# erlgo/openair4G

Hardware: AMD Instinct MI355X
Metric: DL subframes/sec (20 MHz, 2x2, 64-QAM) (higher is better)
Workload: dtype int16; 1 GPU; dlsim 20 MHz 2x2 TM3 (LARGE_CDD) 64-QAM MCS19x2CW, 2x14 IDFT-2048; config_id=C3, global_batch=8192, subframe_index=7, full_grid=False, parallelism=subframe-sharded x1

## Files before the change

include/oai4g.h:

```cpp
#ifndef OAI4G_H
#define OAI4G_H

#include <stddef.h>
#include <stdint.h>

#ifdef __cplusplus
extern "C" {
#endif

#define OAI4G_LTE_NULL 2
#define OAI4G_NSOFT 1827072
#define OAI4G_MAX_SEGMENTS 16
#define OAI4G_MAX_CHANNEL_BITS (14 * 1200 * 6)
#define OAI4G_D_BYTES (96 + 12 + 3 + 3 * 6144)
#define OAI4G_W_BYTES (3 * 6144 + 96)

enum {
  OAI4G_SISO = 0,
  OAI4G_ALAMOUTI = 1,
  OAI4G_LARGE_CDD = 2,
  OAI4G_UNIFORM_PRECODING11 = 3,
  OAI4G_UNIFORM_PRECODING1m1 = 4,
  OAI4G_UNIFORM_PRECODING1j = 5,
  OAI4G_UNIFORM_PRECODING1mj = 6,
// ... 58 lines not shown

typedef struct {
  uint16_t rnti;
  uint8_t current_harq_pid;
  uint8_t Mdlharq;
  uint8_t Kmimo;
  int16_t sqrt_rho_a;
  int16_t sqrt_rho_b;
  oai4g_dl_harq_t *harq_processes[8];
} oai4g_dlsch_t;

int oai4g_init(void);
const char *oai4g_last_error(void);
int oai4g_device_name(char *buf, int len);

int oai4g_init_frame_parms(oai4g_frame_parms_t *fp, uint16_t N_RB_DL, uint16_t Nid_cell, uint8_t Ncp,
                           uint8_t nb_antennas_tx, uint8_t mode1_flag, uint8_t frame_type);
uint8_t oai4g_get_Qm(uint8_t mcs);
int oai4g_get_G(const oai4g_frame_parms_t *fp, uint16_t nb_rb, const uint32_t *rb_alloc, uint8_t mod_order,
                uint8_t Nl, uint8_t num_pdcch_symbols, int frame, uint8_t subframe);
uint8_t oai4g_get_Qm_ul(uint8_t mcs);
uint8_t oai4g_get_I_TBS(uint8_t mcs);
uint8_t oai4g_get_I_TBS_UL(uint8_t mcs);
uint32_t oai4g_tbs_bits(uint8_t I_TBS, uint16_t nb_rb);
uint32_t oai4g_get_TBS_DL(uint8_t mcs, uint16_t nb_rb);
uint32_t oai4g_get_TBS_UL(uint8_t mcs, uint16_t nb_rb);
oai4g_dlsch_t *oai4g_new_dlsch(uint8_t Kmimo, uint8_t Mdlharq, uint8_t N_RB_DL);
void oai4g_free_dlsch(oai4g_dlsch_t *dlsch);
uint32_t oai4g_lte_gold_generic(uint32_t *x1, uint32_t *x2, uint8_t reset);
int oai4g_qpp_fold32(uint32_t K, uint32_t *s, uint16_t *tab);
int oai4g_rsc_scan_rows(uint32_t q, uint32_t rows[6]);
int oai4g_rm_pair_schedule(uint32_t C, uint32_t n0, const uint32_t nt[2], const uint32_t wrapt[2],
                           uint32_t *pairs, uint32_t *pair0);
int oai4g_mod_item_map(uint32_t item, uint32_t ips, uint32_t lz, uint32_t per, uint32_t *sf, uint32_t *l,
                       uint32_t *pair);
uint8_t oai4g_get_pmi(uint8_t N_RB_DL, uint8_t mimo_mode, uint16_t pmi_alloc, uint16_t rb);
void oai4g_set_modofdm_grid_cap(int n_workgroups);

uint32_t oai4g_crc24a(const uint8_t *in, int bitlen);
uint32_t oai4g_crc24b(const uint8_t *in, int bitlen);
int oai4g_lte_segmentation(const uint8_t *input_buffer, uint8_t **output_buffers, uint32_t B, uint32_t *C,
                           uint32_t *Cplus, uint32_t *Cminus, uint32_t *Kplus, uint32_t *Kminus, uint32_t *F);
void oai4g_threegpplte_turbo_encoder(const uint8_t *input, uint16_t input_length_bytes, uint8_t *output,
                                     uint8_t F, uint16_t interleaver_f1, uint16_t interleaver_f2);
uint32_t oai4g_sub_block_interleaving_turbo(uint32_t D, uint8_t *d, uint8_t *w);
uint32_t oai4g_lte_rate_matching_turbo(uint32_t RTC, uint32_t G, const uint8_t *w, uint8_t *e, uint8_t C,
                                       uint32_t Nsoft, uint8_t Mdlharq, uint8_t Kmimo, uint8_t rvidx,
                                       uint8_t Qm, uint8_t Nl, uint8_t r, uint8_t nb_rb, uint8_t m);
int oai4g_dlsch_encoding(uint8_t *a, const oai4g_frame_parms_t *frame_parms, uint8_t num_pdcch_symbols,
                         oai4g_dlsch_t *dlsch, int frame, uint8_t subframe);
void oai4g_dlsch_scrambling(const oai4g_frame_parms_t *frame_parms, int mbsfn_flag, oai4g_dlsch_t *dlsch, int G,
                            uint8_t q, uint8_t Ns);
int oai4g_dlsch_modulation(int32_t **txdataF, int16_t amp, uint32_t subframe_offset,
                           const oai4g_frame_parms_t *frame_parms, uint8_t num_pdcch_symbols,
                           oai4g_dlsch_t *dlsch0, oai4g_dlsch_t *dlsch1);
void oai4g_PHY_ofdm_mod(const int32_t *input, int32_t *output, uint8_t log2fftsize, uint8_t nb_symbols,
                        uint16_t nb_prefix_samples, int etype);
void oai4g_normal_prefix_mod(const int32_t *txdataF, int32_t *txdata, uint8_t nsymb,
                             const oai4g_frame_parms_t *frame_parms);
void oai4g_do_OFDM_mod(int32_t **txdataF, int32_t **txdata, uint32_t frame, uint16_t next_slot,
                       const oai4g_frame_parms_t *frame_parms);
void oai4g_generate_pilots(int32_t **txdataF, int16_t amp, const oai4g_frame_parms_t *frame_parms, uint16_t Ntti);
int oai4g_lte_dl_cell_spec(int32_t *output, int16_t amp, const oai4g_frame_parms_t *frame_parms, uint8_t Ns,
                           uint8_t l, uint8_t p);
int oai4g_idft(int log2n, const int16_t *x, int16_t *y, int scale);
void oai4g_idft2048(const int16_t *x, int16_t *y, int scale);
// ... 260 lines not shown
```

openair4g_amd/__init__.py:

```python
import ctypes
import os

import numpy as np

_HERE = os.path.dirname(os.path.abspath(__file__))
LIB_PATH = os.path.join(_HERE, "lib", "libopenair4g_amd.so")

LTE_NULL = 2
NSOFT = 1827072
MAX_SEGMENTS = 16
MAX_CHANNEL_BITS = 14 * 1200 * 6
D_BYTES = 96 + 12 + 3 + 3 * 6144
W_BYTES = 3 * 6144 + 96
SISO, ALAMOUTI, LARGE_CDD = 0, 1, 2
(UNIFORM_PRECODING11, UNIFORM_PRECODING1m1, UNIFORM_PRECODING1j, UNIFORM_PRECODING1mj, PUSCH_PRECODING0,
 PUSCH_PRECODING1) = 3, 4, 5, 6, 7, 8
CYCLIC_PREFIX = 0


class OAI4GError(RuntimeError):
    pass


u8p = ctypes.POINTER(ctypes.c_uint8)
# ... 271 lines not shown
    "oai4g_tx_config_create": (ctypes.c_void_p, [ctypes.POINTER(TxParams)]),
    "oai4g_tx_config_destroy": (None, [ctypes.c_void_p]),
    "oai4g_tx_G": (ctypes.c_uint32, [ctypes.c_void_p, ctypes.c_int, ctypes.c_int]),
    "oai4g_tx_ebits_words": (ctypes.c_uint32, [ctypes.c_void_p]),
    "oai4g_tx_iq_samples": (ctypes.c_uint32, [ctypes.c_void_p]),
    "oai4g_tx_workspace_bytes": (ctypes.c_size_t, [ctypes.c_void_p, ctypes.c_int]),
    "oai4g_tx_batch": (ctypes.c_int, [ctypes.c_void_p, ctypes.c_int, ctypes.c_void_p, ctypes.c_void_p,
                                      ctypes.c_void_p, ctypes.c_void_p]),
    "oai4g_tx_batch_timed": (ctypes.c_int, [ctypes.c_void_p, ctypes.c_int, ctypes.c_void_p, ctypes.c_void_p,
                                            ctypes.c_void_p, ctypes.c_void_p, ctypes.POINTER(ctypes.c_float)]),
    "oai4g_tx_encode": (ctypes.c_int, [ctypes.c_void_p, ctypes.c_int, ctypes.c_void_p, ctypes.c_void_p,
                                       ctypes.c_void_p]),
    "oai4g_tx_modulate": (ctypes.c_int, [ctypes.c_void_p, ctypes.c_int, ctypes.c_void_p, ctypes.c_void_p,
                                         ctypes.c_void_p]),
    "oai4g_tx_mod_nosat": (ctypes.c_int, [ctypes.c_void_p]),
    "oai4g_diag_encode_phase_ms": (ctypes.c_int, [ctypes.c_void_p, ctypes.c_int, ctypes.c_void_p, ctypes.c_void_p,
                                                  ctypes.c_int, ctypes.c_int, ctypes.POINTER(ctypes.c_float)]),
    "oai4g_diag_encode_occupancy": (ctypes.c_int, [ctypes.c_void_p, ctypes.POINTER(ctypes.c_int),
                                                   ctypes.POINTER(ctypes.c_size_t)]),
    "oai4g_diag_stream": (ctypes.c_int, [ctypes.c_void_p, ctypes.c_void_p, ctypes.c_size_t, ctypes.c_int,
                                         ctypes.c_void_p]),
    "oai4g_dev_alloc": (ctypes.c_void_p, [ctypes.c_size_t]),
    "oai4g_dev_free": (None, [ctypes.c_void_p]),
    "oai4g_memcpy_h2d": (ctypes.c_int, [ctypes.c_void_p, ctypes.c_void_p, ctypes.c_size_t]),
    "oai4g_memcpy_d2h": (ctypes.c_int, [ctypes.c_void_p, ctypes.c_void_p, ctypes.c_size_t]),
    "oai4g_memset_d": (ctypes.c_int, [ctypes.c_void_p, ctypes.c_int, ctypes.c_size_t]),
    "oai4g_sync": (ctypes.c_int, []),
    "oai4g_fill_payload": (ctypes.c_int, [ctypes.c_void_p, ctypes.c_size_t, ctypes.c_uint64, ctypes.c_void_p]),
    "oai4g_qpp_fold32": (ctypes.c_int, [ctypes.c_uint32, ctypes.POINTER(ctypes.c_uint32), ctypes.c_void_p]),
    "oai4g_rsc_scan_rows": (ctypes.c_int, [ctypes.c_uint32, ctypes.POINTER(ctypes.c_uint32)]),
    "oai4g_rm_pair_schedule": (ctypes.c_int, [ctypes.c_uint32, ctypes.c_uint32, ctypes.POINTER(ctypes.c_uint32),
                                              ctypes.POINTER(ctypes.c_uint32), ctypes.POINTER(ctypes.c_uint32),
                                              ctypes.POINTER(ctypes.c_uint32)]),
    "oai4g_mod_item_map": (ctypes.c_int, [ctypes.c_uint32, ctypes.c_uint32, ctypes.c_uint32, ctypes.c_uint32,
                                          ctypes.POINTER(ctypes.c_uint32), ctypes.POINTER(ctypes.c_uint32),
                                          ctypes.POINTER(ctypes.c_uint32)]),
    "oai4g_get_pmi": (ctypes.c_uint8, [ctypes.c_uint8, ctypes.c_uint8, ctypes.c_uint16, ctypes.c_uint16]),
    "oai4g_set_modofdm_grid_cap": (None, [ctypes.c_int]),
    "oai4g_tx_mod_lz": (ctypes.c_int, [ctypes.c_void_p]),
}


def load_library(path=None):
    global _lib
    if _lib is not None:
        return _lib
    path = path or os.environ.get("OAI4G_LIB") or LIB_PATH
    if not os.path.exists(path):
        raise OAI4GError(f"HIP library not built: {path} (run __graft_entry__.build())")
    lib = ctypes.CDLL(path)
    for name, (res, args) in _SIGS.items():
        fn = getattr(lib, name)
        fn.restype = res
        fn.argtypes = args
    _lib = lib
    return lib


def exported_symbols():
    return sorted(_SIGS)


def lib():
    return load_library()


# ... 1045 lines not shown
```

openair4g_amd/csrc/oai4g_encode.hip:

```cpp
#include "oai4g_internal.h"

struct rsc_tables_t {
  uint8_t next[8][16];
  uint8_t par[8][16];
  uint8_t apow[8][8];
  uint32_t hz;
  uint32_t zs[8];
  uint32_t fm[3];
};

static constexpr uint8_t rsc_step_c(uint8_t u, uint8_t s, uint8_t *out)
{
  *out = (uint8_t)((u ^ (s >> 2) ^ (s >> 1)) & 1);
  return (uint8_t)((((u << 2) ^ (s >> 1)) ^ ((s >> 1) << 2) ^ (s << 2)) & 7);
}

static constexpr rsc_tables_t make_rsc_tables()
{
  rsc_tables_t t{};
  for (int s = 0; s < 8; s++)
    for (int nib = 0; nib < 16; nib++) {
      uint8_t st = (uint8_t)s, p = 0;
      for (int b = 0; b < 4; b++) {
        uint8_t o = 0;
// ... 58 lines not shown
  return rsc_parity_of_feedback(rsc_feedback_word(u));
}

[[maybe_unused]] static __device__ __forceinline__ uint32_t rsc_exit_input(uint32_t u)
{
  return (__builtin_popcount(u & k_rsc.fm[0]) & 1u) | ((__builtin_popcount(u & k_rsc.fm[1]) & 1u) << 1) |
         ((__builtin_popcount(u & k_rsc.fm[2]) & 1u) << 2);
}

__constant__ rsc_tables_t c_rsc = k_rsc;



static __device__ __forceinline__ uint32_t bytes_to_seq(uint32_t le) { return __builtin_bswap32(__builtin_bitreverse32(le)); }

static __device__ void crc_table_init(uint32_t *tab, uint32_t poly)
{
  for (uint32_t v = threadIdx.x; v < 256; v += blockDim.x) {
    uint32_t r = v << 16;
    for (int i = 0; i < 8; i++) r = (r & 0x800000u) ? ((r << 1) ^ poly) & 0xffffffu : (r << 1) & 0xffffffu;
    tab[v] = r;
  }
}

static __device__ __forceinline__ void gold_step(uint32_t &x1, uint32_t &x2)
{
  x1 = (x1 >> 1) ^ (x1 >> 4);
  x1 = x1 ^ (x1 << 31) ^ (x1 << 28);
  x2 = (x2 >> 1) ^ (x2 >> 2) ^ (x2 >> 3) ^ (x2 >> 4);
  x2 = x2 ^ (x2 << 31) ^ (x2 << 30) ^ (x2 << 29) ^ (x2 << 28);
}

typedef const __attribute__((address_space(1))) uint32_t gu32_t;

[[maybe_unused]] static __device__ __forceinline__ void gold_generate(uint32_t *gold, uint32_t nwords, uint32_t c_init,
                                                     const uint32_t *gx1, const uint32_t *gx2j)
{
  const uint32_t l = threadIdx.x, w0 = OAI4G_GOLD_STRIDE * l;
  if (l >= OAI4G_GOLD_LANES || w0 >= nwords) return;
  const uint32_t x2i = c_init ^ ((c_init ^ (c_init >> 1) ^ (c_init >> 2) ^ (c_init >> 3)) << 31);
  gu32_t *col = (gu32_t *)(gx2j + l);
  uint32_t cv[32];
#pragma unroll
  for (int b = 0; b < 32; b++) cv[b] = col[OAI4G_GOLD_LANES * b];
  uint32_t x2 = 0;
#pragma unroll
  for (int b = 0; b < 32; b++) x2 ^= cv[b] & (0u - ((x2i >> b) & 1u));
  uint32_t x1 = *(gu32_t *)(gx1 + l);
  const uint32_t wend = min(w0 + OAI4G_GOLD_STRIDE, nwords);
  gold[w0] = x1 ^ x2;
  for (uint32_t w = w0 + 1; w < wend; w++) {
    gold_step(x1, x2);
    gold[w] = x1 ^ x2;
  }
}

static __device__ __forceinline__ uint32_t crc_step(uint32_t reg, uint32_t byte, const uint32_t *tab)
{
  return ((reg << 8) & 0xffffffu) ^ tab[((reg >> 16) ^ byte) & 0xffu];
}

static __device__ __forceinline__ uint32_t crc_mul_tab(uint32_t a, const uint32_t *t )
{
  return t[a & 15u] ^ t[16 + ((a >> 4) & 15u)] ^ t[32 + ((a >> 8) & 15u)] ^ t[48 + ((a >> 12) & 15u)] ^
         t[64 + ((a >> 16) & 15u)] ^ t[80 + ((a >> 20) & 15u)];
}
// ... 427 lines not shown
                                       enc_debug_t dbg, uint32_t *lds_base, int stop_phase = 99, uint32_t sf0 = 0)
{
  const cw_dev_t &cw = c->cw[cwi];
  const uint32_t tid = threadIdx.x, nth = blockDim.x, lane = tid & 63, nwaves = nth >> 6;
  const uint32_t wave = __builtin_amdgcn_readfirstlane(tid >> 6);
  const uint32_t sfi = DEBUG ? sf : (c->first_sf + (sf0 + sf) * c->sf_step) % 10;
  const uint32_t C = __builtin_amdgcn_readfirstlane(cw.C), sw = __builtin_amdgcn_readfirstlane(cw.stream_words);
  uint32_t *strm = lds_base + c->lds_a_words;
  uint32_t *crctab_a = lds_base;
  uint32_t *crctab_b = crctab_a + 256;
  uint32_t *tails = strm + c->lds_b_words;
  uint32_t *crcs = tails + 2 * OAI4G_MAX_CB;
  uint32_t *red = crcs + OAI4G_MAX_CB + 2;
  enc_tabs_t *tabs = (enc_tabs_t *)(red + 4);
  uint32_t *dbg_ebuf = (uint32_t *)(tabs + 1);
  const uint32_t G = cw.G[sfi];

  const uint32_t nw = cw.ilv_off[C], u0 = cw.u0, n0 = cw.n0;
  const uint32_t kw0 = __builtin_amdgcn_readfirstlane(cw.kw[0]), kw1 = __builtin_amdgcn_readfirstlane(cw.kw[1]);
  const uint32_t km0 = __builtin_amdgcn_readfirstlane(cw.kmag[0]), km1 = __builtin_amdgcn_readfirstlane(cw.kmag[1]);
  const uint32_t kk0 = __builtin_amdgcn_readfirstlane(cw.kk[0]), kk1 = __builtin_amdgcn_readfirstlane(cw.kk[1]);
  const uint32_t L8 = __builtin_amdgcn_readfirstlane(cw.L) >> 3, F8 = __builtin_amdgcn_readfirstlane(cw.F) >> 3;
  const uint32_t cb0 = (kk0 >> 3) - L8, cb1 = (kk1 >> 3) - L8;
  auto seg_of = [&](uint32_t r, uint32_t &fill, uint32_t &ncopy, uint32_t &s0) {
    const uint32_t ki = r >= n0 ? 1u : 0u;
    fill = r == 0 ? F8 : 0u;
    ncopy = (ki ? cb1 : cb0) - fill;
    s0 = r == 0 ? 0u : (ki ? n0 * cb0 + (r - n0) * cb1 : r * cb0) - F8;
  };

  const uint8_t *src = payload + (size_t)(DEBUG ? 0 : (sf * c->n_cw + cwi)) * c->payload_stride;
  const uint32_t Ab = cw.A_bytes;
  {
    constexpr uint32_t ENC_BLK = 6;
    const uint32_t nsl = (kw1 + 63) >> 6;
    const uint32_t lim = ((Ab + 3) & ~3u) - 4;
    for (uint32_t sl = wave; sl < nsl; sl += nwaves) {
      const uint32_t j0 = sl << 6, j = j0 + lane, i0 = 4 * j;
      for (uint32_t rb = 0; rb < C; rb += ENC_BLK) {
        uint32_t v[ENC_BLK];
#pragma unroll
        for (uint32_t u = 0; u < ENC_BLK; u++) {
          const uint32_t r = rb + u;
          v[u] = 0;
          if (r >= C) break;
          uint32_t fill, ncopy, s0;
          seg_of(r, fill, ncopy, s0);
          const uint32_t a = s0 + (i0 > fill ? i0 - fill : 0u);
          v[u] = ld_u32_any(src + min(a, lim));
        }
#pragma unroll
        for (uint32_t u = 0; u < ENC_BLK; u++) {
          const uint32_t r = rb + u;
          if (r >= C) break;
          const uint32_t kw = r < n0 ? kw0 : kw1;
          if (j0 >= kw) continue;
          uint32_t fill, ncopy, s0;
          seg_of(r, fill, ncopy, s0);
          const uint32_t nd = s0 + ncopy > Ab ? (Ab > s0 ? Ab - s0 : 0u) : ncopy;
          const uint32_t dend = fill + nd;
          uint32_t *sys = strm + r * 3 * sw;
          if ((sl == 0 && fill != 0) || 4 * (j0 + 64) > dend) {
            if (j < kw) {
              const int pre = (int)fill - (int)i0, valid = (int)dend - (int)i0;
              const uint32_t a = s0 + (pre < 0 ? (uint32_t)-pre : 0u);
              uint32_t le = v[u] >> ((8 * (a - min(a, lim))) & 31u);
              if (pre > 0) le <<= (8 * (uint32_t)pre) & 31u;
              if (valid < 4) le &= (1u << ((8 * (uint32_t)valid) & 31u)) - 1u;
              if (valid <= 0 || pre >= 4) le = 0;
              sys[j] = bytes_to_seq(le);
            }
          } else {
            sys[j] = bytes_to_seq(v[u]);
          }
        }
      }
    }
    for (uint32_t i = tid; i < C * 3 * 4; i += nth) {
      const uint32_t slot = i >> 2, r = slot / 3;
      const uint32_t w = (r < n0 ? kw0 : kw1) + (i & 3u);
      if (w < sw) strm[slot * sw + w] = 0u;
    }
    if (tid == 0) crcs[0] = 0u;
    {
      const uint32_t tv = __builtin_bitreverse32(tid) >> 24, tr = tid & 127u;
      const uint32_t ta = c->crctab[0][tv], tb = c->crctab[1][tv];
      const uint32_t rsc_n = (&c_rsc.next[0][0])[tr], rsc_p = (&c_rsc.par[0][0])[tr];
      const uint32_t rsc_a = (&c_rsc.apow[0][0])[tr & 63u], rsc_z = c_rsc.zs[tr & 7u];
      crctab_a[tid] = __builtin_bitreverse32(ta << 8) << 2;
      if (C > 1) crctab_b[tid] = __builtin_bitreverse32(tb << 8) << 2;
      if (tid < 128) {
        (&tabs->next[0][0])[tid] = (uint8_t)rsc_n;
        (&tabs->par[0][0])[tid] = (uint8_t)rsc_p;
        if (tid < 64) (&tabs->apow[0][0])[tid] = (uint8_t)rsc_a;
        if (tid < 8) tabs->zs[tid] = rsc_z;
      }
    }
  }
  __syncthreads();
  if (stop_phase <= 0) return;

  if (C > 1) {
    const uint32_t lpb = __builtin_amdgcn_readfirstlane(cw.crc_lpb), per = __builtin_amdgcn_readfirstlane(cw.crc_per_cb);
    const uint32_t pos = tid & (lpb - 1);
    for (uint32_t r = tid / lpb; r < C; r += nth / lpb) {
      uint32_t fill, n, s0;
      seg_of(r, fill, n, s0);
      if (s0 + n > Ab) n = Ab > s0 ? Ab - s0 : 0;
// ... 214 lines not shown
          wwalk_init(wk, p, R, Kpi);
          w[p] = wwalk_null(wk, R, ND) ? OAI4G_LTE_NULL : (uint8_t)wwalk_bit(wk, blk, sw, tails, r, K, ND, Kpi);
        }
      }
    }
    if (!dbg.e) return;
  }

  const uint32_t nd0 = __builtin_amdgcn_readfirstlane(cw.NDk[0]), nd1 = __builtin_amdgcn_readfirstlane(cw.NDk[1]);
  for (uint32_t r = tid; r < C; r += nth) {
    const uint32_t K = r < n0 ? kk0 : kk1, ND = r < n0 ? nd0 : nd1;
    uint32_t *blk = strm + r * 3 * sw;
    for (uint32_t s = 0; s < 3; s++) {
      uint32_t t4 = tail_bit(tails, r, s) | (tail_bit(tails, r, 3 + s) << 1) | (tail_bit(tails, r, 6 + s) << 2) |
                    (tail_bit(tails, r, 9 + s) << 3);
      uint32_t w0 = K >> 5, off = K & 31;
      blk[s * sw + w0] |= t4 << off;
      if (off > 28) blk[s * sw + (w0 + 1)] |= t4 >> (32 - off);
    }
    if (ND == 0) blk[2 * sw + ((K + 4) >> 5)] |= (blk[2 * sw] & 1u) << ((K + 4) & 31u);
  }
  __syncthreads();

  {
    const tp_lane_t tpl = tp_lane(tid & 31);
    const uint32_t sw3 = __builtin_amdgcn_readfirstlane(3 * sw);
    const uint32_t Nnn0 = __builtin_amdgcn_readfirstlane(cw.Nnnk[0]), Nnn1 = __builtin_amdgcn_readfirstlane(cw.Nnnk[1]);
    bool once;
    {
      const uint32_t Elo = __builtin_amdgcn_readfirstlane(cw.E[sfi][0]), Ehi = __builtin_amdgcn_readfirstlane(cw.E[sfi][C - 1]);
      const uint32_t wrapt0 = __builtin_amdgcn_readfirstlane(cw.rm_wrapt[0]), wrapt1 = __builtin_amdgcn_readfirstlane(cw.rm_wrapt[1]);
      once = Ehi <= min(Nnn0, Nnn1) && Elo <= min(Nnn0, Nnn1) && wrapt0 != ~1u && wrapt1 != ~1u;
    }
    typedef const __attribute__((address_space(4))) uint32_t cu32_t;
    cu32_t *pdesc = (cu32_t *)cw.rm_pairs, *ppair0 = (cu32_t *)cw.rm_pair0;
    cu32_t *pE = (cu32_t *)cw.E[sfi], *proff = (cu32_t *)cw.roff[sfi];
    gu32_t *gold = (gu32_t *)(c->gold_tab + (size_t)(sfi * c->n_cw + cwi) * c->ebits_words);
    uint32_t *eout = DEBUG ? nullptr : ebits + (size_t)(sf * c->n_cw + cwi) * c->ebits_words;
    uint32_t *ebuf = DEBUG ? dbg_ebuf : lds_base;
    const uint32_t hb = DEBUG ? C : (C + 1) >> 1, nhalf = DEBUG ? 1u : 2u;
    uint32_t carry = 0;
    for (uint32_t h = 0; h < nhalf; h++) {
      const uint32_t rb0 = h ? hb : 0, rb1 = h ? C : hb;
      const uint32_t eb0 = proff[rb0], eb1 = rb1 < C ? proff[rb1] : G;
      const uint32_t w0 = eb0 >> 5, nwh = ((eb1 + 31) >> 5) - w0;
      for (uint32_t i = tid; i < nwh + 1; i += nth) ebuf[i] = (i == 0 && h) ? carry : 0u;
      __syncthreads();
      const uint32_t pb = ppair0[rb0], pe = ppair0[rb1], bit0 = 32 * w0;
      const char *rsrc0 = (const char *)&cw.rm_src[0][0][0], *rdst0 = (const char *)&cw.rm_dst[0][0][0];
      auto pair_loop = [&](auto ONCE) {
        uint32_t P = pb + wave;
        if (P >= pe) return;
        const uint32_t plast = pe - 1;
        uint32_t d = pdesc[P], dn = pdesc[min(P + nwaves, plast)];
        uint32_t E, ro, nsrc, ndst;
        auto fetch = [&]() {
          E = pE[(d >> 2) & 15u];
          ro = proff[(d >> 2) & 15u];
          nsrc = *(const uint32_t *)(rsrc0 + ((d >> 16) + 4 * lane));
          ndst = *(const uint32_t *)(rdst0 + ((d >> 16) + 4 * lane));
        };
        fetch();
        for (;;) {
          const uint32_t src = nsrc, dst = ndst, dc = d, Ec = E, rob = ro - bit0;
          d = dn;
          dn = pdesc[min(P + 2 * nwaves, plast)];
          fetch();
// ... 9 lines not shown
            if (dc & 1u) {
              asm volatile("" ::: "memory");
              if (dst & OAI4G_RM_DST_WRAP) {
                const uint32_t ma = ((dc & 2u) ? Nnn1 : Nnn0) - o;
                const uint32_t l2 = min(m - ma, Ec);
                or_bits2(ebuf, rob, (y >> ma) & (0xffffffffu >> (32 - l2)));
              }
            }
          } else if (m) {
            const uint32_t Nnn = (dc & 2u) ? Nnn1 : Nnn0;
            y &= 0xffffffffu >> (32 - m);
            const uint32_t ma = min(m, Nnn - o);
            for (uint32_t part = 0; part < 2; part++) {
              const uint32_t len = part ? m - ma : ma, os = part ? 0u : o;
              const uint32_t v = part ? (ma < 32 ? y >> ma : 0u) : (ma < 32 ? y & ((1u << ma) - 1u) : y);
              for (uint32_t x = os; len && x < Ec; x += Nnn) {
                const uint32_t l = min(len, Ec - x);
                or_bits(ebuf, rob + x, v & (0xffffffffu >> (32 - l)));
              }
            }
          }
          P += nwaves;
          if (P >= pe) break;
        }
      };
      if (once) pair_loop(std::true_type{});
      else pair_loop(std::false_type{});
      __syncthreads();
      if (DEBUG) {
        for (uint32_t k = tid; k < G; k += nth) dbg.e[k] = (uint8_t)((ebuf[k >> 5] >> (k & 31)) & 1u);
        return;
      }
      const uint32_t nst = stop_phase <= 4 ? 0u : ((h + 1 < nhalf && (eb1 & 31u)) ? nwh - 1 : nwh);
      for (uint32_t i = tid; i < nst; i += nth) {
        const uint32_t wi = w0 + i;
        uint32_t v = ebuf[i] ^ gold[wi];
        const uint32_t nb = min(32u, G - 32 * wi);
        if (nb < 32) v &= (1u << nb) - 1u;
        eout[wi] = v;
      }
      if (h + 1 < nhalf) {
        carry = (eb1 & 31u) ? ebuf[nwh - 1] : 0u;
        __syncthreads();
      }
    }
  }
}

__global__ void __launch_bounds__(256) __attribute__((amdgpu_num_sgpr(80))) k_encode(const cfg_dev_t *__restrict__ c, const uint8_t *__restrict__ payload,
                                                uint32_t *__restrict__ ebits, int stop_phase, uint32_t sf0)
{
  extern __shared__ uint32_t lds_dyn[];
  uint32_t sf = blockIdx.x / c->n_cw, cwi = blockIdx.x % c->n_cw;
  enc_debug_t none = {nullptr, nullptr, nullptr, nullptr, nullptr};
  encode_codeword<false>(c, sf, cwi, payload, ebits, none, lds_dyn, stop_phase, sf0);
}

__global__ void __launch_bounds__(256) k_encode_debug(const cfg_dev_t *__restrict__ c, uint32_t sf, uint32_t cwi,
                                                      const uint8_t *__restrict__ payload, enc_debug_t dbg)
{
  extern __shared__ uint32_t lds_dyn[];
  encode_codeword<true>(c, sf, cwi, payload, nullptr, dbg, lds_dyn);
}

static size_t enc_lds_bytes(const cfg_dev_t *h)
{
  size_t words = (size_t)h->lds_a_words + h->lds_b_words + 2 * OAI4G_MAX_CB + OAI4G_MAX_CB + 2 + 4;
  size_t bytes = words * 4 + sizeof(enc_tabs_t);
#ifdef OAI4G_ENC_LDS_PAD
  bytes += OAI4G_ENC_LDS_PAD;
#endif
  return (bytes + 15) & ~(size_t)15;
}
// ... 253 lines not shown
```

openair4g_amd/csrc/oai4g_host.cpp:

```cpp
#include <hip/hip_runtime.h>
#include <math.h>
#include <pthread.h>
#include <stdarg.h>
#include <stdio.h>
#include <stdlib.h>
#include <string.h>

#include <algorithm>
#include <cmath>
#include <cstdlib>
#include <vector>
#include <map>
#include <mutex>
#include <vector>

#include "../../include/oai4g.h"
#include "../../include/oai4g_qpp.h"
#include "../../include/oai4g_tbs.h"
#include "oai4g_internal.h"

static thread_local char g_err[512] = "";

static void set_err(const char *fmt, ...)
{
// ... 705 lines not shown
      if (il && L == 31 && ND > 0 && left <= 32 && n) n--;
      const uint32_t z = rb ? 0u : zc, ci0 = rb ? cs + 32 * rb - zc : cs, p0 = pc + 32 * rb;
      const int m = p0 + (uint32_t)n > Ncb ? (int)Ncb - (int)(p0 + z) : n - (int)z;
      if (m <= 0) continue;
      uint32_t o = ci0 + Nnn - k0c;
      o = o >= Nnn ? o - Nnn : o;
      c.rm_dst[ki][t][L] = o | (z << 16) | ((uint32_t)m << 21) | (o + (uint32_t)m > Nnn ? OAI4G_RM_DST_WRAP : 0u);
      if (o + (uint32_t)m > Nnn) c.rm_wrapt[ki] = c.rm_wrapt[ki] == ~0u || c.rm_wrapt[ki] == t ? t : ~1u;
    }
  }
  if (getenv("OAI4G_ENC_GENERAL_RM")) c.rm_wrapt[ki] = ~1u;
}

extern "C" int oai4g_rm_pair_schedule(uint32_t C, uint32_t n0, const uint32_t nt[2], const uint32_t wrapt[2],
                                      uint32_t *pairs, uint32_t *pair0)
{
  if (C < 1 || C > OAI4G_MAX_CB || n0 > C) return -1;
  for (uint32_t ki = 0; ki < 2; ki++)
    if ((ki ? n0 < C : n0 > 0) && (nt[ki] < 1 || nt[ki] > OAI4G_RM_TILES)) return -1;
  uint32_t n = 0;
  for (uint32_t r = 0; r < C; r++) {
    const uint32_t ki = r >= n0 ? 1u : 0u, pp = (nt[ki] + 1) / 2;
    pair0[r] = n;
    for (uint32_t p = 0; p < pp; p++) {
      const uint32_t t0 = 2 * p, row = ki * ((OAI4G_RM_TILES + 1) * 32) + t0 * 32;
      const uint32_t wrap = wrapt[ki] - t0 < 2u ? 1u : 0u;
      pairs[n++] = wrap | (ki << 1) | (r << 2) | ((4 * row) << 16);
    }
  }
  pair0[C] = n;
  return (int)n;
}

extern "C" int oai4g_qpp_fold32(uint32_t K, uint32_t *s_out, uint16_t *tab)
{
  const int qi = oai4g_qpp_index(K);
  if (qi < 0 || oai4g_qpp_table[qi].K != K) return -1;
  if (K & 1023u) return 0;
  const uint64_t f1 = oai4g_qpp_table[qi].f1, f2 = oai4g_qpp_table[qi].f2;
  const uint32_t Q = K >> 5;
  auto pi = [&](uint64_t k) { return (uint32_t)((f1 * k + f2 * k * k) % K); };
  const uint32_t d = (pi(Q) + K - pi(0)) % K;
  if (d % Q) return 0;
  const uint32_t s = d / Q;
  if (!(s & 1u)) return 0;
  for (uint32_t k = 0; k < K; k++)
    if ((pi(k + Q) + K - pi(k)) % K != d) return 0;
  uint32_t si = 1;
  while (((si * s) & 31u) != 1u) si += 2;
  *s_out = s;
  for (uint32_t k = 0; k < Q; k++) {
    const uint32_t x = pi(k);
    tab[k] = (uint16_t)(((x % Q) << 7) | ((si * (x / Q)) & 31u));
  }
  return 1;
}

static int derive_cfg(oai4g_tx_config *cfg, const oai4g_tx_params_t *p, const uint8_t Nl[2], bool need_remap,
                      int only_sf)
{
  memset(&cfg->h, 0, sizeof(cfg->h));
  cfg->p = *p;
  oai4g_frame_parms_t &fp = cfg->fp;
  if (oai4g_init_frame_parms(&fp, p->N_RB_DL, p->Nid_cell, p->Ncp, p->nb_antennas_tx, p->mode1_flag,
                             p->frame_type) != 0)
    return -1;
// ... 189 lines not shown
    c.wpk_off[C] = wwords;
    c.ntask = ntask;
    for (uint32_t r = 0; r < C; r++) {
      const uint32_t ki = r < c.n0 ? 0 : 1;
      if (c.K[r] != c.kk[ki]) { set_err("block size order"); return -1; }
      c.Rk[ki] = c.R[r]; c.NDk[ki] = c.ND[r]; c.Ncbk[ki] = c.Ncb[r]; c.Nnnk[ki] = c.Nnn[r]; c.k0ck[ki] = c.k0c[r];
    }
    for (uint32_t r = 0; r < C; r++) {
      const uint32_t ki = r < c.n0 ? 0 : 1;
      if (c.R[r] != c.Rk[ki] || c.ND[r] != c.NDk[ki] || c.Ncb[r] != c.Ncbk[ki] || c.Nnn[r] != c.Nnnk[ki] ||
          c.k0c[r] != c.k0ck[ki] || c.kidx[r] != ki) {
        set_err("per-size block geometry differs");
        return -1;
      }
    }
    if (c.n0 == 0) { c.Rk[0] = c.Rk[1]; c.NDk[0] = c.NDk[1]; c.Ncbk[0] = c.Ncbk[1]; c.Nnnk[0] = c.Nnnk[1]; c.k0ck[0] = c.k0ck[1]; }
    for (int ki = 0; ki < 2; ki++) {
      c.nullcol[ki][0] = c.nullcol[ki][1] = 0;
      for (uint32_t wc = 0; wc < 32; wc++) {
        uint32_t pc = 0;
        for (int b = 0; b < 5; b++) pc |= ((wc >> b) & 1u) << (4 - b);
        if (pc < c.NDk[ki]) c.nullcol[ki][0] |= 1u << wc;
        if (pc + 1 < c.NDk[ki]) c.nullcol[ki][1] |= 1u << wc;
      }
      c.t0k[ki] = (c.Rk[ki] + 31) / 32;
      c.ntk[ki] = c.t0k[ki] + (c.Rk[ki] + 15) / 16;
      c.ntmag[ki] = ((1u << 20) + c.ntk[ki] - 1) / c.ntk[ki];
      if (c.ntk[ki] > OAI4G_RM_TILES) { set_err("rate-matching plan: %u tiles", c.ntk[ki]); return -1; }
      rm_plan(c, ki);
    }
    if (oai4g_rm_pair_schedule(C, c.n0, c.ntk, c.rm_wrapt, c.rm_pairs, c.rm_pair0) < 0) {
      set_err("rate-matching pair schedule");
      return -1;
    }
    max_w = wwords > max_w ? wwords : max_w;
    uint32_t tbw = (c.A_bytes + 3 + 3) / 4 + 1;
    max_tb_words = tbw > max_tb_words ? tbw : max_tb_words;
    uint32_t strw = C * 3 * c.stream_words;
    max_stream_words = strw > max_stream_words ? strw : max_stream_words;
    for (int sf = 0; sf < 10; sf++) {
      int G;
      if (fp.nb_antennas_tx == 4) {
        std::vector<uint16_t> tmp((size_t)14 * fp.ofdm_symbol_size);
        uint32_t sb[14];
        int n = build_remap(&fp, p->rb_alloc, p->num_pdcch_symbols, sf, p->mimo_mode, (uint16_t)p->pmi_alloc, tmp.data(), sb,
                            nullptr);
        G = n < 0 ? -1 : n * (int)c.Qm;
      } else {
        G = oai4g_get_G(&fp, p->nb_rb, p->rb_alloc, (uint8_t)c.Qm, Nl[cw], p->num_pdcch_symbols, 0, (uint8_t)sf);
      }
      if (G <= 0 || G > OAI4G_MAX_CHANNEL_BITS) { set_err("G=%d out of range", G); return -1; }
      c.G[sf] = (uint32_t)G;
      uint32_t Gp = (uint32_t)G / Nl[cw] / c.Qm, GpmodC = Gp % C, off = 0;
      for (uint32_t r = 0; r < C; r++) {
        uint32_t E = (r < C - GpmodC) ? Nl[cw] * c.Qm * (Gp / C) : Nl[cw] * c.Qm * ((GpmodC ? 1 : 0) + Gp / C);
        c.E[sf][r] = E;
        c.roff[sf][r] = off;
        off += E;
      }
      c.roff[sf][C] = off;
      c.esplit[sf] = C - GpmodC;
      for (int h = 0; h < 2; h++) {
        const uint32_t E = c.E[sf][h ? C - 1 : 0], w = (E + 31) / 32;
        c.ew[sf][h] = w;
        c.emag[sf][h] = w ? (uint32_t)(((1ull << 32) + w - 1) / w) : 0u;
      }
// ... 3249 lines not shown
```

openair4g_amd/csrc/oai4g_internal.h:

```cpp
#pragma once
#include <hip/hip_runtime.h>
#include <stdint.h>

#include "../../include/oai4g.h"

#define OAI4G_MAX_CB 16
#define OAI4G_MAX_NULLS 104
#define OAI4G_MAX_CHUNKS 192
#define OAI4G_MAX_TASKS (OAI4G_MAX_CB * 20)
#define OAI4G_RM_TILES 20
#define OAI4G_RM_SRC_LAST (1u << 20)
#define OAI4G_RM_DST_WRAP (1u << 27)
#define OAI4G_PIPE_MAX_CHUNKS 16
#define OAI4G_CRS_CODE 0xE000u
#define OAI4G_CTL_CODE 0xC000u
static constexpr uint32_t oai4g_mod_entry_shift(uint32_t mimo_mode, uint32_t n_ant, uint32_t log2N)
{
  return log2N != 11 ? 1u : mimo_mode == OAI4G_LARGE_CDD && n_ant == 2 ? 3u : mimo_mode == OAI4G_SISO ? 2u : 1u;
}
static constexpr uint32_t oai4g_mod_addr_mask(uint32_t shift) { return 0x7FFFu & ~((1u << shift) - 1u); }
static constexpr uint32_t oai4g_mod_sentinel(uint32_t N) { return (3u * N) / 4u; }
static constexpr bool oai4g_mode_prec1(uint32_t mimo_mode)
{
  return mimo_mode >= OAI4G_UNIFORM_PRECODING11 && mimo_mode <= OAI4G_PUSCH_PRECODING1;
}
#define OAI4G_MOD_PMI_SHIFT 12u
static constexpr uint32_t oai4g_mod_pmi_bits = 3u << OAI4G_MOD_PMI_SHIFT;
static constexpr uint32_t oai4g_mod_pmi_idx_mask = (1u << OAI4G_MOD_PMI_SHIFT) - 1u;
static_assert(2u * (oai4g_mod_sentinel(2048) + 4u) <= (1u << OAI4G_MOD_PMI_SHIFT), "staged offsets must stay below the precoder bits");
static constexpr bool oai4g_mod_nre_fits(uint32_t nre, uint32_t N) { return nre + 3u <= oai4g_mod_sentinel(N); }
struct oai4g_mod_item_t {
  uint32_t sf, l, pair;
};
static constexpr uint32_t oai4g_mod_permag(uint32_t per) { return (uint32_t)(((1ull << 32) + per - 1) / per); }
static inline __host__ __device__ oai4g_mod_item_t oai4g_mod_item(uint32_t item, uint32_t ips, uint32_t lz, uint32_t per,
                                                                  uint32_t permag)
{
  const uint32_t it = item / ips;
  const uint32_t sf = (uint32_t)(((uint64_t)it * permag) >> 32);
  return {sf, lz + it - sf * per, item - it * ips};
}
#define OAI4G_MOD_LZ_MAX 4u
#define OAI4G_ENC_CRC_TABLE_WORDS (256 + 256)
// ... 42 lines not shown
  uint32_t ntask;
  uint16_t tasks[OAI4G_MAX_TASKS];
  uint32_t ilv_off[OAI4G_MAX_CB + 1];
  uint32_t qpp0[2][OAI4G_MAX_CHUNKS];
  alignas(16) uint32_t qpp_tab[2][OAI4G_MAX_CHUNKS * 4];
  uint32_t qpp_f32[2];
  uint32_t qpp_s3[2];
  uint32_t n0, u0, kk[2], kw[2], kmag[2];
  uint32_t Rk[2], NDk[2], Ncbk[2], Nnnk[2], k0ck[2];
  uint32_t ntk[2], t0k[2], ntmag[2];
  uint32_t rm_wrapt[2];
  uint32_t nullcol[2][2];
  uint32_t esplit[10], ew[10][2], emag[10][2];
  uint32_t nnull[2];
  uint16_t nullpos[2][OAI4G_MAX_NULLS];
  uint32_t G[10];
  uint32_t E[10][OAI4G_MAX_CB];
  uint32_t roff[10][OAI4G_MAX_CB + 1];
  int16_t qam_a[8], qam_b[8];
  int16_t qpsk_a, qpsk_b;
  int16_t alm_qpsk[2][2];
  uint32_t stream_words;
  uint32_t crc_per_tb;
  uint32_t crc_per_cb;
  uint32_t crc_lpb;
  uint32_t crcmul_tb[8][6][16];
  uint32_t crcmul_blk[OAI4G_MAX_CB][96];
  uint32_t crc2_tb[2][8][96];
  uint32_t crc2_cb[2][2][8][96];
  uint32_t rm_src[2][OAI4G_RM_TILES + 1][32];
  uint32_t rm_dst[2][OAI4G_RM_TILES + 1][32];
  uint32_t rm_pair0[OAI4G_MAX_CB + 1];
  uint32_t rm_pairs[OAI4G_MAX_CB * ((OAI4G_RM_TILES + 1) / 2)];
};

struct cfg_dev_t {
  uint32_t N_RB_DL, N, log2N, cp0, cp, spt, nsymb, n_ant, first_carrier;
  uint32_t n_cw, mimo_mode, num_pdcch, rnti, Nid_cell, first_sf, sf_step;
  uint32_t payload_stride;
  uint32_t ebits_words;
  uint32_t lds_tb_words;
  uint32_t lds_stream_words;
  uint32_t lds_gold_words;
  uint32_t lds_w_words;
  uint32_t lds_a_words;
  uint32_t lds_b_words;
  uint32_t mod_nosat;
  uint32_t mod_lz, mod_per, mod_permag;
  uint32_t crctab[2][256];
  cw_dev_t cw[2];
  uint32_t symbase[10][14];
  uint32_t symnre[10][14];
  uint32_t n_cu;
  const uint16_t *remap;
  const uint16_t *remap_tm;
  uint32_t with_crs;
  uint32_t pilmask;
  uint32_t ctlmask[10];
  uint32_t ctl_on;
  const uint32_t *gold_tab;
  const uint32_t *gold_x1;
  const uint32_t *gold_x2j;
  const uint32_t *tw;
  const uint32_t *stat_tm;
  uint32_t stat_planes;
  uint32_t pad2;
// ... 222 lines not shown
```

Before: 9.468 million subframes/s.

## Precompute payload slab schedule on host and flatten encoder copy loop

```diff
diff --git a/include/oai4g.h b/include/oai4g.h
--- a/include/oai4g.h
+++ b/include/oai4g.h
@@ -114,6 +114,8 @@
 int oai4g_rsc_scan_rows(uint32_t q, uint32_t rows[6]);
 int oai4g_rm_pair_schedule(uint32_t C, uint32_t n0, const uint32_t nt[2], const uint32_t wrapt[2],
                            uint32_t *pairs, uint32_t *pair0);
+int oai4g_enc_slab_schedule(uint32_t C, uint32_t n0, const uint32_t kk[2], uint32_t L, uint32_t F,
+                            uint32_t A_bytes, uint32_t sw, uint32_t *units);
 int oai4g_mod_item_map(uint32_t item, uint32_t ips, uint32_t lz, uint32_t per, uint32_t *sf, uint32_t *l,
                        uint32_t *pair);
 uint8_t oai4g_get_pmi(uint8_t N_RB_DL, uint8_t mimo_mode, uint16_t pmi_alloc, uint16_t rb);
diff --git a/openair4g_amd/__init__.py b/openair4g_amd/__init__.py
--- a/openair4g_amd/__init__.py
+++ b/openair4g_amd/__init__.py
@@ -327,6 +327,9 @@
     "oai4g_rm_pair_schedule": (ctypes.c_int, [ctypes.c_uint32, ctypes.c_uint32, ctypes.POINTER(ctypes.c_uint32),
                                               ctypes.POINTER(ctypes.c_uint32), ctypes.POINTER(ctypes.c_uint32),
                                               ctypes.POINTER(ctypes.c_uint32)]),
+    "oai4g_enc_slab_schedule": (ctypes.c_int, [ctypes.c_uint32, ctypes.c_uint32, ctypes.POINTER(ctypes.c_uint32),
+                                               ctypes.c_uint32, ctypes.c_uint32, ctypes.c_uint32, ctypes.c_uint32,
+                                               ctypes.POINTER(ctypes.c_uint32)]),
     "oai4g_mod_item_map": (ctypes.c_int, [ctypes.c_uint32, ctypes.c_uint32, ctypes.c_uint32, ctypes.c_uint32,
                                           ctypes.POINTER(ctypes.c_uint32), ctypes.POINTER(ctypes.c_uint32),
                                           ctypes.POINTER(ctypes.c_uint32)]),
diff --git a/openair4g_amd/csrc/oai4g_encode.hip b/openair4g_amd/csrc/oai4g_encode.hip
--- a/openair4g_amd/csrc/oai4g_encode.hip
+++ b/openair4g_amd/csrc/oai4g_encode.hip
@@ -114,6 +114,7 @@
 }
 
 typedef const __attribute__((address_space(1))) uint32_t gu32_t;
+typedef const __attribute__((address_space(4))) uint32_t cu32_t;
 
 [[maybe_unused]] static __device__ __forceinline__ void gold_generate(uint32_t *gold, uint32_t nwords, uint32_t c_init,
                                                      const uint32_t *gx1, const uint32_t *gx2j)
@@ -607,48 +608,43 @@
   const uint8_t *src = payload + (size_t)(DEBUG ? 0 : (sf * c->n_cw + cwi)) * c->payload_stride;
   const uint32_t Ab = cw.A_bytes;
   {
-    constexpr uint32_t ENC_BLK = 6;
-    const uint32_t nsl = (kw1 + 63) >> 6;
+    constexpr uint32_t ENC_UNITS = (OAI4G_ENC_SLABS * 13 + 3) / 4;
+    cu32_t *pun = (cu32_t *)&cw.enc_units[0][0];
+    const uint32_t nun = __builtin_amdgcn_readfirstlane(cw.enc_nunits);
     const uint32_t lim = ((Ab + 3) & ~3u) - 4;
-    for (uint32_t sl = wave; sl < nsl; sl += nwaves) {
-      const uint32_t j0 = sl << 6, j = j0 + lane, i0 = 4 * j;
-      for (uint32_t rb = 0; rb < C; rb += ENC_BLK) {
-        uint32_t v[ENC_BLK];
-#pragma unroll
-        for (uint32_t u = 0; u < ENC_BLK; u++) {
-          const uint32_t r = rb + u;
-          v[u] = 0;
-          if (r >= C) break;
-          uint32_t fill, ncopy, s0;
-          seg_of(r, fill, ncopy, s0);
-          const uint32_t a = s0 + (i0 > fill ? i0 - fill : 0u);
-          v[u] = ld_u32_any(src + min(a, lim));
+    const uint32_t lane4 = 4 * lane;
+    uint32_t v[ENC_UNITS];
+#pragma unroll
+    for (uint32_t u = 0; u < ENC_UNITS; u++) {
+      const uint32_t un = wave + u * nwaves;
+      v[u] = 0;
+      if (un >= nun) break;
+      const uint32_t d0 = pun[2 * un], d1 = pun[2 * un + 1];
+      const uint32_t s0 = d0 & 0xffffu, fill = (d1 >> 15) & 7u, i0 = lane4 + ((d1 >> 5) & 0x300u);
+      const uint32_t a = s0 + (i0 > fill ? i0 - fill : 0u);
+      v[u] = ld_u32_any(src + min(a, lim));
+    }
+#pragma unroll
+    for (uint32_t u = 0; u < ENC_UNITS; u++) {
+      const uint32_t un = wave + u * nwaves;
+      if (un >= nun) break;
+      const uint32_t d0 = pun[2 * un], d1 = pun[2 * un + 1];
+      uint32_t *sys = strm + (d1 & 0x1fffu);
+      const uint32_t j = ((d1 >> 7) & 0xc0u) + lane;
+      if (d0 & OAI4G_ENC_UNIT_EXACT) {
+        const uint32_t kw = (d1 >> 18) & 0xffu;
+        if (j < kw) {
+          const uint32_t s0 = d0 & 0xffffu, dend = (d0 >> 16) & 0xfffu, fill = (d1 >> 15) & 7u, i0 = 4 * j;
+          const int pre = (int)fill - (int)i0, valid = (int)dend - (int)i0;
+          const uint32_t a = s0 + (pre < 0 ? (uint32_t)-pre : 0u);
+          uint32_t le = v[u] >> ((8 * (a - min(a, lim))) & 31u);
+          if (pre > 0) le <<= (8 * (uint32_t)pre) & 31u;
+          if (valid < 4) le &= (1u << ((8 * (uint32_t)valid) & 31u)) - 1u;
+          if (valid <= 0 || pre >= 4) le = 0;
+          sys[j] = bytes_to_seq(le);
         }
-#pragma unroll
-        for (uint32_t u = 0; u < ENC_BLK; u++) {
-          const uint32_t r = rb + u;
-          if (r >= C) break;
-          const uint32_t kw = r < n0 ? kw0 : kw1;
-          if (j0 >= kw) continue;
-          uint32_t fill, ncopy, s0;
-          seg_of(r, fill, ncopy, s0);
-          const uint32_t nd = s0 + ncopy > Ab ? (Ab > s0 ? Ab - s0 : 0u) : ncopy;
-          const uint32_t dend = fill + nd;
-          uint32_t *sys = strm + r * 3 * sw;
-          if ((sl == 0 && fill != 0) || 4 * (j0 + 64) > dend) {
-            if (j < kw) {
-              const int pre = (int)fill - (int)i0, valid = (int)dend - (int)i0;
-              const uint32_t a = s0 + (pre < 0 ? (uint32_t)-pre : 0u);
-              uint32_t le = v[u] >> ((8 * (a - min(a, lim))) & 31u);
-              if (pre > 0) le <<= (8 * (uint32_t)pre) & 31u;
-              if (valid < 4) le &= (1u << ((8 * (uint32_t)valid) & 31u)) - 1u;
-              if (valid <= 0 || pre >= 4) le = 0;
-              sys[j] = bytes_to_seq(le);
-            }
-          } else {
-            sys[j] = bytes_to_seq(v[u]);
-          }
-        }
+      } else {
+        sys[j] = bytes_to_seq(v[u]);
       }
     }
     for (uint32_t i = tid; i < C * 3 * 4; i += nth) {
@@ -929,7 +925,6 @@
       const uint32_t wrapt0 = __builtin_amdgcn_readfirstlane(cw.rm_wrapt[0]), wrapt1 = __builtin_amdgcn_readfirstlane(cw.rm_wrapt[1]);
       once = Ehi <= min(Nnn0, Nnn1) && Elo <= min(Nnn0, Nnn1) && wrapt0 != ~1u && wrapt1 != ~1u;
     }
-    typedef const __attribute__((address_space(4))) uint32_t cu32_t;
     cu32_t *pdesc = (cu32_t *)cw.rm_pairs, *ppair0 = (cu32_t *)cw.rm_pair0;
     cu32_t *pE = (cu32_t *)cw.E[sfi], *proff = (cu32_t *)cw.roff[sfi];
     gu32_t *gold = (gu32_t *)(c->gold_tab + (size_t)(sfi * c->n_cw + cwi) * c->ebits_words);
@@ -1005,13 +1000,10 @@
         return;
       }
       const uint32_t nst = stop_phase <= 4 ? 0u : ((h + 1 < nhalf && (eb1 & 31u)) ? nwh - 1 : nwh);
-      for (uint32_t i = tid; i < nst; i += nth) {
-        const uint32_t wi = w0 + i;
-        uint32_t v = ebuf[i] ^ gold[wi];
-        const uint32_t nb = min(32u, G - 32 * wi);
-        if (nb < 32) v &= (1u << nb) - 1u;
-        eout[wi] = v;
-      }
+      const bool shortw = h + 1 == nhalf && (G & 31u) && nst;
+      const uint32_t nfull = shortw ? nst - 1 : nst;
+      for (uint32_t i = tid; i < nfull; i += nth) eout[w0 + i] = ebuf[i] ^ gold[w0 + i];
+      if (shortw && tid == (nfull & (nth - 1))) eout[w0 + nfull] = (ebuf[nfull] ^ gold[w0 + nfull]) & ((1u << (G & 31u)) - 1u);
       if (h + 1 < nhalf) {
         carry = (eb1 & 31u) ? ebuf[nwh - 1] : 0u;
         __syncthreads();
diff --git a/openair4g_amd/csrc/oai4g_host.cpp b/openair4g_amd/csrc/oai4g_host.cpp
--- a/openair4g_amd/csrc/oai4g_host.cpp
+++ b/openair4g_amd/csrc/oai4g_host.cpp
@@ -761,6 +761,32 @@
   return (int)n;
 }
 
+extern "C" int oai4g_enc_slab_schedule(uint32_t C, uint32_t n0, const uint32_t kk[2], uint32_t L, uint32_t F,
+                                       uint32_t A_bytes, uint32_t sw, uint32_t *units)
+{
+  if (C < 1 || C > OAI4G_MAX_CB || n0 > C || (L != 0 && L != 24) || F >= 64 || (F & 7u)) return -1;
+  for (uint32_t ki = 0; ki < 2; ki++)
+    if ((ki ? n0 < C : n0 > 0) && (kk[ki] < 40 || kk[ki] > 6144 || (kk[ki] & 7u) || (kk[ki] + 31) / 32 + 3 > sw)) return -1;
+  if (C * 3 * sw >= (1u << 13) || A_bytes >= (1u << 16)) return -1;
+  const uint32_t L8 = L >> 3, F8 = F >> 3, cb[2] = {(kk[0] >> 3) - L8, (kk[1] >> 3) - L8};
+  uint32_t n = 0;
+  for (uint32_t r = 0; r < C; r++) {
+    const uint32_t ki = r >= n0 ? 1u : 0u, kw = (kk[ki] + 31) / 32;
+    const uint32_t fill = r == 0 ? F8 : 0u, ncopy = cb[ki] - fill;
+    const uint32_t s0 = r == 0 ? 0u : (ki ? n0 * cb[0] + (r - n0) * cb[1] : r * cb[0]) - F8;
+    const uint32_t nd = s0 + ncopy > A_bytes ? (A_bytes > s0 ? A_bytes - s0 : 0u) : ncopy;
+    const uint32_t dend = fill + nd;
+    if (s0 >= (1u << 16)) return -1;
+    for (uint32_t sl = 0; 64 * sl < kw; sl++) {
+      const bool exact = (sl == 0 && fill != 0) || 4 * (64 * sl + 64) > dend;
+      units[2 * n] = s0 | (dend << 16) | (exact ? OAI4G_ENC_UNIT_EXACT : 0u);
+      units[2 * n + 1] = (r * 3 * sw) | (sl << 13) | (fill << 15) | (kw << 18);
+      n++;
+    }
+  }
+  return (int)n;
+}
+
 extern "C" int oai4g_qpp_fold32(uint32_t K, uint32_t *s_out, uint16_t *tab)
 {
   const int qi = oai4g_qpp_index(K);
@@ -1016,6 +1042,11 @@
     if (oai4g_rm_pair_schedule(C, c.n0, c.ntk, c.rm_wrapt, c.rm_pairs, c.rm_pair0) < 0) {
       set_err("rate-matching pair schedule");
       return -1;
+    }
+    {
+      const int nu = oai4g_enc_slab_schedule(C, c.n0, c.kk, c.L, c.F, c.A_bytes, c.stream_words, &c.enc_units[0][0]);
+      if (nu < 0) { set_err("payload slab schedule"); return -1; }
+      c.enc_nunits = (uint32_t)nu;
     }
     max_w = wwords > max_w ? wwords : max_w;
     uint32_t tbw = (c.A_bytes + 3 + 3) / 4 + 1;
diff --git a/openair4g_amd/csrc/oai4g_internal.h b/openair4g_amd/csrc/oai4g_internal.h
--- a/openair4g_amd/csrc/oai4g_internal.h
+++ b/openair4g_amd/csrc/oai4g_internal.h
@@ -9,6 +9,8 @@
 #define OAI4G_MAX_CHUNKS 192
 #define OAI4G_MAX_TASKS (OAI4G_MAX_CB * 20)
 #define OAI4G_RM_TILES 20
+#define OAI4G_ENC_SLABS 3
+#define OAI4G_ENC_UNIT_EXACT (1u << 31)
 #define OAI4G_RM_SRC_LAST (1u << 20)
 #define OAI4G_RM_DST_WRAP (1u << 27)
 #define OAI4G_PIPE_MAX_CHUNKS 16
@@ -117,6 +119,8 @@
   uint32_t rm_dst[2][OAI4G_RM_TILES + 1][32];
   uint32_t rm_pair0[OAI4G_MAX_CB + 1];
   uint32_t rm_pairs[OAI4G_MAX_CB * ((OAI4G_RM_TILES + 1) / 2)];
+  uint32_t enc_nunits;
+  alignas(8) uint32_t enc_units[OAI4G_MAX_CB * OAI4G_ENC_SLABS][2];
 };
 
 struct cfg_dev_t {
```

Result: no change. 9.562 million subframes/s, median of 6 (+1.0%).
